# okgarces/deep-successor-features-for-transfer

Hardware: AMD Instinct MI355X
Metric: env steps/sec (whole node), Reacher 8-task SF-DQN at 1/2/4/8 MI355X (higher is better)
Workload: dtype fp32; 1 GPU; reacher17-all-T8-B32 (Reacher-shape |s|=17 |a|=7 d=8, psi MLP 256x2, all heads updated per env step: main_sfdqn_torch.py path); heads_per_gpu=8, heads_total=8, global_batch=32, replay=host, parallelism=single

## Files before the change

deep-successor-features-for-transfer_amd/csrc/sfx.hip:

```cpp
#include <hip/hip_ext.h>
#include <hip/hip_runtime.h>
#include <dlfcn.h>
#include <rccl/rccl.h>

#include <cmath>
#include <cstdio>
#include <cstdlib>
#include <cstring>
#include <algorithm>
#include <atomic>
#include <chrono>
#include <deque>
#include <map>
#include <random>
#include <string>
#include <functional>
#include <tuple>
#include <utility>
#include <vector>

#include "sfx_kernels.h"
#include "sfx_gpiw.h"
#include "sfx_tsf.h"
#include "sfx_phi.h"
// ... 38 lines not shown
      all = all && f != nullptr;
    };
    sym(a.GetUniqueId, "ncclGetUniqueId");
    sym(a.CommInitRank, "ncclCommInitRank");
    sym(a.AllReduce, "ncclAllReduce");
    sym(a.CommDestroy, "ncclCommDestroy");
    sym(a.CommAbort, "ncclCommAbort");
    sym(a.CommGetAsyncError, "ncclCommGetAsyncError");
    sym(a.CommSplit, "ncclCommSplit");
    sym(a.CommCount, "ncclCommCount");
    sym(a.CommUserRank, "ncclCommUserRank");
    sym(a.GetErrorString, "ncclGetErrorString");
    a.ok = all;
    if (!all) a.why = "RCCL lacks a needed entry point";
    return a;
  }();
  return api;
}

#define SFX_FAIL(code, msg) \
  do {                      \
    g_err = (msg);          \
    return (code);          \
  } while (0)

#define HIPCHK(x)                                                     \
  do {                                                                \
    hipError_t e_ = (x);                                              \
    if (e_ != hipSuccess) {                                           \
      g_err = std::string(#x) + ": " + hipGetErrorString(e_);         \
      return SFX_E_HIP;                                               \
    }                                                                 \
  } while (0)

#define LAUNCHCHK()                                                   \
  do {                                                                \
    hipError_t e_ = hipGetLastError();                                \
    if (e_ != hipSuccess) {                                           \
      g_err = std::string("kernel launch: ") + hipGetErrorString(e_); \
      return SFX_E_HIP;                                               \
    }                                                                 \
  } while (0)

#define RC(x)            \
  do {                   \
    int rc_ = (x);       \
    if (rc_) return rc_; \
  } while (0)

namespace {

inline int align4(int x) { return (x + 3) & ~3; }
inline int align8(int x) { return (x + 7) & ~7; }
inline int cdiv(int a, int b) { return (a + b - 1) / b; }

struct GraphKey {
  int op, a0, a1, a2, a3, a4, a5, a6;
  unsigned long long mask;
  const void* p[12];
  bool operator<(const GraphKey& o) const { return std::memcmp(this, &o, sizeof(GraphKey)) < 0; }
};

struct StepOut {
  int64_t sel[2];
  int flag;
  unsigned done;
  int posted;
  int pad_;
};

}

struct sfx_handle {
  int T = 0, n_s = 0, H = 0, nh = 0, A = 0, d = 0, O = 0, NL = 0, Mmax = 0, device = 0;
  int P = 0, Ptorch = 0, dpad = 0, actSize = 0;
  std::vector<LayerGeo> L;
  std::vector<int> actOff;
  hipStream_t stream = nullptr;
  hipStream_t cap = nullptr;
  bool use_graphs = true;
  int fwd_tpw = FWD_TPW;
  SelScratch* selk = nullptr;
  int ncu = 256;
  AdamHP hp_psi{1e-3, 0.0, 0.9, 0.999, 1e-8};
  AdamHP hp_w{1e-3, 0.0, 0.9, 0.999, 1e-8};
  int target_update_ev = 1000;
  std::vector<int> since_target, host_step;
  unsigned long long mask = 0;
  std::map<GraphKey, hipGraphExec_t> graphs;
  std::map<GraphKey, bool> graph_posts;
  std::map<GraphKey, int> keys_seen;
  long long graph_eager = 0;
  Geo G{};
  bool prof = false;
  struct ProfRec {
    int kind;
    double bytes;
    hipEvent_t a, b;
  };
  std::vector<ProfRec> prof_recs;
  std::vector<hipEvent_t> prof_pool;
  bool lazy_finish = false;
  struct Pending {
    bool active = false, update = false, sel = false;
    int B = 0, use_gpi = 1, task = 0, sel_use_gpi = 1;
    const float *S = nullptr, *S1 = nullptr, *phi = nullptr, *gamma = nullptr, *s_next = nullptr;
    const int64_t* a = nullptr;
    float* losses = nullptr;
    bool pre = false;
    const float* ax = nullptr;
    int aM = 0;
    bool posted = false;
    float* q_out = nullptr;
    int64_t* task_out = nullptr;
    const unsigned long long* out_ind = nullptr;
  } pend;
  long long steps_spec = 0, steps_fallback = 0, policies_rerun = 0, rounds_total = 0;
  long long graph_captures = 0, graph_launches = 0;
  int force_rerun_from = -1;
  int spec_rounds = 2;
  bool spec_rounds_auto = true;
  int Tg = 0, off = 0;
  struct sfx_tsf_state* tsf = nullptr;
  struct sfx_phi_state* phi = nullptr;
  int comm_rank = 0, comm_world = 0;
  ncclComm_t comm = nullptr;
  bool comm_owned = false;
  ncclComm_t comm_rounds = nullptr;
  bool rounds_comm = false;
  bool comm_dead = false;
  std::string comm_err;
  long long* dstall = nullptr;
  bool comm_force = false;
  int (*host_ar)(void*, int32_t*, int) = nullptr;
  void* host_ar_ctx = nullptr;
  int32_t* host_ar_buf = nullptr;
  size_t host_ar_cap = 0;
  int *xb[2] = {nullptr, nullptr}, *xge = nullptr;
  int *tsx = nullptr, *tsz = nullptr;
  int *qh = nullptr, *qhs = nullptr;
  bool shard_qa = true;
  Pending spend;

  float *online = nullptr, *target = nullptr, *am = nullptr, *av = nullptr;
  float *w = nullptr, *wm = nullptr, *wv = nullptr;
  int* step = nullptr;
  int* dcancel = nullptr;
  AdamC* adamc = nullptr;
  float *act = nullptr, *dz = nullptr, *rowloss = nullptr;
  int64_t* spec_next = nullptr;
  int* skip = nullptr;
  unsigned long long* skipc = nullptr;
  bool skip_rounds = true;
  bool bwd_merge = true;
  int tdg_rows = 0;
  StepOut* dout = nullptr;
  HostResult* pub_res = nullptr;
  const long long* pub_dctr = nullptr;
  bool pub_folded = false;
  bool fold_publish = true;
  bool bf16 = false;
  __bf16* on16 = nullptr;
  __bf16* tg16 = nullptr;
  int dxs_max = 1, dx_ntile = 1;
  float* dxpart = nullptr;
  unsigned* dxctr = nullptr;
// ... 172 lines not shown
    F.K = L.K;
    F.act = L.actOut;
    F.wOff = L.wOff;
    F.bOff = L.bOff;
    F.xOff = l == 0 || l0 ? -1 : h->actOff[l - 1];
    F.yOff = h->actOff[l];
    F.w0Off = h->L[0].wOff;
    F.b0Off = h->L[0].bOff;
    F.K0 = h->L[0].K;
    F.y0Off = h->actOff[0];
    const bool first = l == ex.l0 || l0;
    F.lms_head = first ? ex.lms_head : -1;
    F.lms_phi = ex.lms_phi;
    F.lms_r = ex.lms_r;
    F.lms_r_ind = first ? ex.lms_r_ind : nullptr;
    F.lms_alpha = ex.lms_alpha;
    F.flag = first ? ex.flag : nullptr;
    F.flag_value = ex.flag_value;
    const bool qa = ex.qa_role >= 0 && l == h->NL - 1;
    const bool aligned = l > 0 || ((uintptr_t)xa % 16 == 0 && (uintptr_t)xb % 16 == 0);
    bool own = false;
    if (F.xcd)
      for (const FwdGroup& g : groups) own = own || (g.m > 0 && g.m != M);
    F.ntN = cdiv(L.N, 16);
    long tiles32 = 0;
    for (const FwdGroup& g : groups) tiles32 += (long)F.ntN * cdiv(own && g.m > 0 ? g.m : M, 32) * g.n;
    F.tail = !l0 && !qa && (L.K % 32) == 0 && aligned && own && tiles32 > h->ncu ? 1 : 0;
    F.ntM = fwd_row_tiles(M, F.tail);
    F.tpw = 1;
    long tiles = (long)F.ntN * F.ntM * ninst;
    F.rowsplit = 0;
    if (own) {
      int* mt[4] = {&F.mt0, &F.mt1, &F.mt2, &F.mt3};
      int gi = 0;
      F.ntMs = 0;
      tiles = 0;
      for (const FwdGroup& g : groups) {
        *mt[gi++] = fwd_row_tiles(g.m > 0 ? g.m : M, F.tail);
        F.ntMs += *mt[gi - 1];
        tiles += (long)F.ntN * *mt[gi - 1] * g.n;
      }
      F.rowsplit = 1;
    }
    if (qa) {
      F.qa_role = ex.qa_role;
      F.qa_Tg = h->Tg;
      F.qa_off = h->off;
      F.qa_M = ex.qa_M;
      F.qa_all = ex.qa_all;
      F.qa_ge = ex.qa_ge;
      F.qa_lt = ex.qa_lt;
      F.qa_sel = ex.qa_sel;
      F.qa_row = ex.qa_row;
      F.qa_task = ex.qa_task;
      F.qa_use_gpi = ex.qa_use_gpi;
      F.qh = ex.qh;
      F.qhs = ex.qhs;
    }
    if (!qa && h->fwd_tpw > 1 && F.ntN > 1 && 2 * tiles >= 3L * h->ncu && (tiles <= 4L * h->ncu || F.rowsplit) &&
        (l0 || ((L.K % 32) == 0 && aligned)))
      F.tpw = h->fwd_tpw;
    const int ntNb = cdiv(F.ntN, F.tpw);
    const dim3 grid = F.xcd ? dim3(8 * cdiv(h->T, 8) * ntNb * (F.rowsplit ? F.ntMs : F.ntM * F.ngroups))
                            : dim3(ntNb, ninst, F.ntM);
    double by = 0.0;
    for (const FwdGroup& g : groups) {
      const double m = g.m > 0 ? g.m : M;
      by += 4.0 * g.n * ((double)L.N * L.K + L.N + m * L.K + m * L.N);
      if (l0) by += 4.0 * g.n * ((double)h->L[0].N * h->L[0].K + h->L[0].N + m * h->L[0].K);
    }
    const bool tp2 = F.tpw > 1;
    const bool gemv = !l0 && !qa && M <= GEMV_M && L.N >= GEMV_N && L.K % 16 == 0 &&
                      (l > 0 || ((uintptr_t)xa % 16 == 0 && (uintptr_t)xb % 16 == 0));
    if (gemv) {
      launch(h, K_FWD, by, k_fwd_gemv, dim3(cdiv(L.N, 64), ninst), dim3(256), h->G, F);
    } else if (l0) {
      if (!(ex.ride_l0 && !F.xcd && ex.ride_l0(F, grid, by)))
        launch(h, K_FWD, by,
               tp2 ? (h->bf16 ? k_fwd<true, true, true, 2> : k_fwd<true, true, false, 2>)
                   : (h->bf16 ? k_fwd<true, true, true> : k_fwd<true, true>),
               grid, dim3(64 * FWD_WAVES), h->G, F);
    } else {
      const bool vec = (L.K % 32) == 0 && aligned;
      launch(h, K_FWD, by,
             !vec ? k_fwd<false, false>
                  : tp2 ? (h->bf16 ? k_fwd<true, false, true, 2> : k_fwd<true, false, false, 2>)
                        : (h->bf16 ? k_fwd<true, false, true> : k_fwd<true, false>),
             grid, dim3(64 * FWD_WAVES), h->G, F);
    }
  }
  LAUNCHCHK();
  return SFX_OK;
}

bool wide_gpi(const sfx_handle* h) {
  return (long)h->T * h->A > 256 && h->d % 4 == 0 && h->d <= 16 && h->A <= WAMAX;
}

#define SFX_WIDE(K) (h->d == 4 ? K<1> : h->d == 8 ? K<2> : h->d == 12 ? K<3> : K<4>)

int run_tdg(sfx_handle* h, int pol0, int npol, int guess, int M, int use_gpi, const int64_t* a, const float* phi,
            const float* gamma, int64_t* next, int next_stride, int* flag = nullptr, const int* xmax = nullptr,
            int poloff = 0, const float* dz_scale = nullptr, const int64_t* prev = nullptr, bool skip = false) {
  const double nt = use_gpi ? h->T : 1;
  const double by = 4.0 * npol * M * (nt * h->O + 2.0 * h->O + 2.0 * h->d + 4);
  if (use_gpi && !xmax && !dz_scale && wide_gpi(h)) {
    TdgwArgs W{};
    W.M = M;
    W.pol0 = pol0;
    W.npol = npol;
    W.guess = guess;
    W.next_stride = next_stride;
    W.flag_value = h->T;
    W.a = a;
    W.phi = phi;
    W.gamma = gamma;
    W.next = next;
    W.flag = flag;
    W.prev = skip ? prev : nullptr;
    W.skip = skip ? h->skip : nullptr;
    W.skipc = skip ? h->skipc : nullptr;
    launch(h, K_TDG, by, SFX_WIDE(k_tdgw), dim3(M, cdiv(npol, WPC)), dim3(256), h->G, W);
    LAUNCHCHK();
    return SFX_OK;
  }
  TdgArgs A{};
  A.dz_scale = dz_scale;
  A.xmax = xmax;
  A.poloff = poloff;
  A.M = M;
  A.use_gpi = use_gpi;
  A.pol0 = pol0;
  A.npol = npol;
  A.guess = guess;
  A.flag = flag;
  A.flag_value = h->T;
  A.next_stride = next_stride;
  A.a = a;
  A.phi = phi;
  A.gamma = gamma;
  A.next = next;
  A.prev = skip ? prev : nullptr;
  A.skip = skip ? h->skip : nullptr;
  A.skipc = skip ? h->skipc : nullptr;
  launch(h, K_TDG, by, k_tdg, dim3(M, npol), dim3(256), h->G, A);
  LAUNCHCHK();
  return SFX_OK;
}

struct TdgSpec {
  int use_gpi = 1, guess = R_S1, next_stride = 0;
  const int64_t* a = nullptr;
  const float* gamma = nullptr;
  int64_t* next = nullptr;
  int* flag = nullptr;
  const int* xmax = nullptr;
  int poloff = 0;
  const int* xi_src = nullptr;
  int* xi_dst = nullptr;
  int xi_copy = 0, xi_n = 0;
  const int64_t* prev = nullptr;
  bool skip = false;
  const float* dz_scale = nullptr;
};

int tdg_variant(const sfx_handle* h) {
  if ((h->d & 3) != 0 || h->O > TDG_ROWS_O || h->A > 128) return 0;
  const long ta = (long)h->T * h->A;
// ... 688 lines not shown
                          float* phi_copy, const int64_t* idx, const float* gam, int B, float* S, float* PHI, float* S1,
                          int64_t* A, float* G, int n_s, int d) {
  if (!rs || !rphi || !rs1 || !ra || j < 0 || !s || !phi || !s1 || !a || !idx || (!rg && !gam) || B < 1 || !S ||
      !PHI || !S1 || !A || !G || n_s < 1 || d < 1)
    SFX_FAIL(SFX_E_ARG, "sfx_replay_put_gather: bad arguments");
  const PutGather P{rs, rphi, rs1, ra, rg, j, s, phi, s1, a, s1_copy, phi_copy, idx, gam, S, PHI, S1, G, A, B, n_s, d};
  hipLaunchKernelGGL(k_replay_put_gather, dim3(B + 1), dim3(64), 0, (hipStream_t)stream, P);
  LAUNCHCHK();
  return SFX_OK;
}
const char* sfx_last_error(void) { return g_err.c_str(); }

int sfx_check_failures(long long* count, long long* first_host, int reset) {
  if (!count) SFX_FAIL(SFX_E_ARG, "null argument");
#ifdef SFX_CHECK
  unsigned n = 0;
  HIPCHK(hipDeviceSynchronize());
  HIPCHK(hipMemcpyFromSymbol(&n, HIP_SYMBOL(sfx::g_chk_n), sizeof(n)));
  if (first_host) HIPCHK(hipMemcpyFromSymbol(first_host, HIP_SYMBOL(sfx::g_chk_rec), sizeof(long long) * 32));
  if (reset) {
    const unsigned z = 0;
    HIPCHK(hipMemcpyToSymbol(HIP_SYMBOL(sfx::g_chk_n), &z, sizeof(z)));
  }
  *count = n;
#else
  (void)first_host;
  (void)reset;
  *count = -1;
#endif
  return SFX_OK;
}

#ifdef SFX_PROBE
int sfx_probe_dump(void* out_host, int max_recs) {
  unsigned n = 0;
  if (hipDeviceSynchronize() != hipSuccess) return -1;
  if (hipMemcpyFromSymbol(&n, HIP_SYMBOL(sfx::g_probe_n), sizeof(n)) != hipSuccess) return -1;
  if (n > sfx::PROBE_N) n = sfx::PROBE_N;
  if ((int)n > max_recs) n = (unsigned)max_recs;
  if (n && hipMemcpyFromSymbol(out_host, HIP_SYMBOL(sfx::g_probe), n * sizeof(sfx::ProbeRec)) != hipSuccess) return -1;
  const unsigned z = 0;
  if (hipMemcpyToSymbol(HIP_SYMBOL(sfx::g_probe_n), &z, sizeof(z)) != hipSuccess) return -1;
  return (int)n;
}
#endif

int sfx_create(sfx_t* out, int T, int n_s, int H, int n_hidden, const int* acts, int A, int d, int max_batch,
               int device, void* stream) {
  if (!out) SFX_FAIL(SFX_E_ARG, "out is null");
  *out = nullptr;
  if (T < 1 || T > 64 || n_s < 1 || H < 1 || n_hidden < 0 || n_hidden + 2 > NLMAX || A < 1 || d < 1 ||
      max_batch < 1)
    SFX_FAIL(SFX_E_ARG, "bad geometry (1 <= T <= 64 heads per handle)");
  if (d > DMAX || max_batch + 1 > MMAX || A > AMAX || (long)T * A > QMAX || (long)A * d > OMAX)
    SFX_FAIL(SFX_E_ARG, "geometry exceeds kernel limits (d<=256, batch<1024, A<=256, T*A<=8192, A*d<=4096)");
  for (int i = 0; i < n_hidden; ++i)
    if (!acts || acts[i] < ACT_NONE || acts[i] > ACT_TANH) SFX_FAIL(SFX_E_ARG, "bad activation code");
  HIPCHK(hipSetDevice(device));
  sfx_handle* h = new sfx_handle();
  h->T = T;
  h->n_s = n_s;
  h->H = H;
  h->nh = n_hidden;
  h->A = A;
  h->d = d;
  h->O = A * d;
  h->NL = n_hidden + 2;
  h->Mmax = max_batch;
  h->device = device;
  h->stream = (hipStream_t)stream;
  h->dpad = align4(d);
  const char* eg = std::getenv("SFX_GRAPHS");
  h->use_graphs = !(eg && eg[0] == '0');
  const char* efp = std::getenv("SFX_FOLD_PUBLISH");
  h->fold_publish = !(efp && efp[0] == '0');
  {
    int dev = 0, ncu = 0;
    if (hipGetDevice(&dev) == hipSuccess &&
        hipDeviceGetAttribute(&ncu, hipDeviceAttributeMultiprocessorCount, dev) == hipSuccess && ncu > 0)
      h->ncu = ncu;
  }
  const char* etp = std::getenv("SFX_FWD_TPW");
  h->fwd_tpw = etp && etp[0] == '1' ? 1 : FWD_TPW;
  const char* eqa = std::getenv("SFX_SHARD_QA");
  h->shard_qa = !(eqa && eqa[0] == '0');
  const char* esk = std::getenv("SFX_SKIP");
  h->skip_rounds = !(esk && esk[0] == '0');
  const char* ebm = std::getenv("SFX_BWD_MERGE");
  h->bwd_merge = !(ebm && ebm[0] == '0');
  const char* etr = std::getenv("SFX_TDG_ROWS");
  const int tr = etr ? std::atoi(etr) : 0;
  h->tdg_rows = tr == 16 || tr == 32 ? tr : 0;
  int off = 0, ptorch = 0;
  for (int l = 0; l < h->NL; ++l) {
    LayerGeo Lr{};
    if (l == 0) {
      Lr.N = H; Lr.K = n_s; Lr.actOut = ACT_NONE;
    } else if (l == h->NL - 1) {
      Lr.N = h->O; Lr.K = H; Lr.actOut = ACT_NONE;
    } else {
      Lr.N = H; Lr.K = H; Lr.actOut = acts[l - 1];
    }
    Lr.actIn = l > 0 ? h->L[l - 1].actOut : ACT_NONE;
    Lr.wOff = align8(off);
    off = Lr.wOff + Lr.N * Lr.K;
    Lr.bOff = align4(off);
    off = Lr.bOff + Lr.N;
    ptorch += Lr.N * Lr.K + Lr.N;
    h->L.push_back(Lr);
  }
  h->P = (off + 63) & ~63;
  h->Ptorch = ptorch;
  int aoff = 0;
  for (int l = 0; l < h->NL; ++l) {
    h->actOff.push_back(aoff);
    aoff += align4((max_batch + 1) * h->L[l].N);
  }
  h->actSize = (aoff + 63) & ~63;
  h->Tg = T;
  h->spec_rounds = auto_spec_rounds(T);
  h->since_target.assign(T, 0);
  h->host_step.assign(T, 0);

  const size_t headBytes = sizeof(float) * (size_t)T * h->P;
  const size_t wBytes = sizeof(float) * (size_t)T * h->dpad;
  int rc = SFX_OK;
  auto alloc = [&](void** p, size_t bytes) {
    if (rc != SFX_OK) return;
    if (hipMalloc(p, bytes) != hipSuccess || hipMemset(*p, 0, bytes) != hipSuccess) {
      g_err = "hipMalloc failed";
      rc = SFX_E_HIP;
    }
  };
  alloc((void**)&h->online, 2 * headBytes);
  alloc((void**)&h->target, headBytes);
  alloc((void**)&h->am, 2 * headBytes);
  alloc((void**)&h->av, 2 * headBytes);
  alloc((void**)&h->w, wBytes);
  alloc((void**)&h->wm, wBytes);
  alloc((void**)&h->wv, wBytes);
  alloc((void**)&h->step, sizeof(int) * T);
  alloc((void**)&h->dcancel, 64);
  alloc((void**)&h->adamc, sizeof(AdamC) * T);
  {
    int nmax = 0, kmax = 0;
    for (const LayerGeo& L : h->L) {
      nmax = std::max(nmax, L.N);
      kmax = std::max(kmax, L.K);
    }
    h->dxs_max = std::max(1, cdiv(nmax, DX_SPLIT_N));
    h->dx_ntile = cdiv(max_batch, 32) * cdiv(kmax, 16);
    if (h->dxs_max > 1) {
      alloc((void**)&h->dxpart, sizeof(float) * 512 * (size_t)T * h->dx_ntile * h->dxs_max);
      alloc((void**)&h->dxctr, sizeof(unsigned) * (size_t)T * h->dx_ntile);
    }
  }
  alloc((void**)&h->act, sizeof(float) * (size_t)NROLE * T * h->actSize);
  alloc((void**)&h->dz, sizeof(float) * (size_t)T * h->actSize);
  alloc((void**)&h->rowloss, sizeof(float) * (size_t)T * MMAX);
  alloc((void**)&h->spec_next, sizeof(int64_t) * 2 * (size_t)T * MMAX);
  alloc((void**)&h->skip, sizeof(int) * 2 * (size_t)T);
  alloc((void**)&h->skipc, 64);
  alloc((void**)&h->dout, sizeof(StepOut));
  alloc((void**)&h->selk, sizeof(SelScratch));
  if (rc == SFX_OK &&
      hipHostMalloc((void**)&h->hout, sizeof(StepOut), hipHostMallocCoherent | hipHostMallocMapped) != hipSuccess) {
// ... 640 lines not shown
```

deep-successor-features-for-transfer_amd/csrc/sfx_kernels.h:

```cpp
#pragma once
#include <hip/hip_runtime.h>
#include <stdint.h>

#include <type_traits>

namespace sfx {

typedef float floatx4 __attribute__((ext_vector_type(4)));

constexpr int NLMAX = 8;
constexpr int MT = 32;
constexpr int QMAX = 8192;
constexpr int OMAX = 4096;
constexpr int AMAX = 256;
constexpr int DMAX = 256;
constexpr int MMAX = 1024;
constexpr int KFUSE = 64;
constexpr int GEMV_N = 512;
constexpr int GEMV_M = 4;
constexpr int DX_SPLIT_N = 256;
constexpr int VFUSE = 4096;
constexpr int TQF = 4096;

enum { ACT_NONE = 0, ACT_RELU = 1, ACT_TANH = 2 };
// ... 312 lines not shown
    for (int k = 0; k < d; ++k) q = __builtin_fmaf(p[k], w[k], q);
    const int v = sortable(q);
    SFX_CHK(i < Tg && m0 + bl < F.qa_M && head < G.T, i, m0 + bl, head);
    const size_t o = ((size_t)i * F.qa_M + m0 + bl) * Aa + a;
    if (all) atomicMax(F.qa_all + o, v);
    if (ge) atomicMax(F.qa_ge + o, v);
    if (lt) atomicMax(F.qa_lt + o, v);
    if (F.qh) F.qh[(((size_t)head * Tg + i) * F.qa_M + m0 + bl) * Aa + a] = v;
  }
  const int rl = F.qa_row - m0;
  if ((F.qa_sel || F.qhs) && rl >= 0 && rl < 32 && (F.qa_use_gpi || tg == F.qa_task))
    for (int al = tid; al < na; al += nt) {
      const int a = a0 + al;
      if (a >= Aa) continue;
      const float* p = sT + rl * 16 + al * d;
      const float* w = sw + F.qa_task * d;
      float q = 0.f;
      for (int k = 0; k < d; ++k) q = __builtin_fmaf(p[k], w[k], q);
      const int v = sortable(q);
      if (F.qa_sel) F.qa_sel[(size_t)tg * Aa + a] = v;
      if (F.qhs) F.qhs[(size_t)head * Aa + a] = v;
    }
}

__device__ void q_replay(const Geo& G, const FwdArgs& F, int head, int tN, int tM) {
  const int d = G.d, Aa = G.A, Tg = F.qa_Tg, tid = threadIdx.x, nt = blockDim.x;
  const int n0 = tN * 16, m0 = tM * 32, na = 16 / d, a0 = n0 / d, tg = F.qa_off + head;
  const int mrows = F.qa_M - m0 < 32 ? F.qa_M - m0 : 32;
  const int per_i = (mrows > 0 ? mrows : 0) * na;
  for (int it = tid; it < Tg * per_i; it += nt) {
    const int i = it / per_i, rem = it - i * per_i, bl = rem / na, al = rem - bl * na, a = a0 + al;
    if (a >= Aa || !F.qa_lt || tg >= i) continue;
    const int v = F.qh[(((size_t)head * Tg + i) * F.qa_M + m0 + bl) * Aa + a];
    atomicMax(F.qa_lt + ((size_t)i * F.qa_M + m0 + bl) * Aa + a, v);
  }
  const int rl = F.qa_row - m0;
  if (F.qa_sel && rl >= 0 && rl < 32 && (F.qa_use_gpi || tg == F.qa_task))
    for (int al = tid; al < na; al += nt) {
      const int a = a0 + al;
      if (a < Aa) F.qa_sel[(size_t)tg * Aa + a] = F.qhs[(size_t)head * Aa + a];
    }
}

__device__ void lms_apply(float* w, const float* phi, const float* r, float alpha, int d, int cx) {
  __shared__ float s_p[DMAX];
  __shared__ float s_e;
  const int tid = threadIdx.x;
  const float wk = tid < d ? w[tid] : 0.f, pk = tid < d ? phi[tid] : 0.f;
  if (tid < d) s_p[tid] = __fmul_rn(pk, wk);
  __syncthreads();
  if (tid == 0) {
    float rf = 0.f;
    for (int k = 0; k < d; ++k) rf = __fadd_rn(rf, s_p[k]);
    s_e = __fmul_rn(alpha, __fsub_rn(r[0], rf));
  }
  __syncthreads();
  if (tid < d && !cx) w[tid] = __fadd_rn(wk, __fmul_rn(s_e, pk));
}

__device__ void lms_block(const Geo& G, const FwdArgs& F) {
  const float* r = F.lms_r_ind ? reinterpret_cast<const float*>(F.lms_r_ind[0]) : F.lms_r;
  lms_apply(G.w + (long long)F.lms_head * G.dpad, F.lms_phi, r, F.lms_alpha, G.d, step_cancelled(G.cancel));
}

constexpr int L0_KMAX = 64, L0_NMAX = 256;

__device__ __forceinline__ FwdGroup fwd_group(const FwdArgs& F, int& y) {
  int gs = 0;
  if (F.ngroups > 1 && y >= F.g0.n) { y -= F.g0.n; gs = 1; }
  if (F.ngroups > 2 && gs == 1 && y >= F.g1.n) { y -= F.g1.n; gs = 2; }
  if (F.ngroups > 3 && gs == 2 && y >= F.g2.n) { y -= F.g2.n; gs = 3; }
  auto pick = [gs](int a, int b, int c, int d) { return gs == 0 ? a : gs == 1 ? b : gs == 2 ? c : d; };
  FwdGroup g;
  g.role = pick(F.g0.role, F.g1.role, F.g2.role, F.g3.role);
  g.which = pick(F.g0.which, F.g1.which, F.g2.which, F.g3.which);
  g.xsel = pick(F.g0.xsel, F.g1.xsel, F.g2.xsel, F.g3.xsel);
  g.head0 = pick(F.g0.head0, F.g1.head0, F.g2.head0, F.g3.head0);
  g.n = pick(F.g0.n, F.g1.n, F.g2.n, F.g3.n);
  g.m = pick(F.g0.m, F.g1.m, F.g2.m, F.g3.m);
  g.noskip = pick(F.g0.noskip, F.g1.noskip, F.g2.noskip, F.g3.noskip);
  return g;
}

constexpr int FWD_TPW = 2;
constexpr int FWD_WAVES = 8;

__host__ __device__ __forceinline__ int fwd_row_tiles(int m, int tail) {
  return tail && m > 32 ? (m + 15) >> 5 : (m + 31) >> 5;
}

template <bool VEC, bool L0, bool BF = false, int TP = 1>
__device__ __forceinline__ void fwd_tile(const Geo& G, const FwdArgs& F, int y, int tN, int tM, float* sT = nullptr) {
  constexpr int TPW = TP;
  static_assert(TP == 1 || VEC, "several tiles per workgroup: vector tiles only");
  const int ntile = TP == 1 ? 1 : (F.ntN - tN < F.tpw ? F.ntN - tN : F.tpw);
  static_assert(!BF || VEC, "bf16 operands: vector tiles only");
  constexpr int KW = 256 / FWD_WAVES;
  constexpr int KL = KW / 4;
  const FwdGroup grp = fwd_group(F, y);
  const int head = grp.head0 + y;
  const int M = grp.m > 0 ? grp.m : F.M, N = F.N, K = F.K;
  if (tM >= fwd_row_tiles(M, F.tail)) return;
  const float* P = grp.which == P_TARGET ? G.target + (long long)head * G.P
                                         : G.online + G.slot_off(rslot(F.mask, head) ^ (grp.which == P_NEW), head);
  const float* X = F.xOff < 0 ? (grp.xsel == 1 ? F.xa : grp.xsel == 2 ? F.xb : F.xc) : G.actp(grp.role, head, F.xOff);
  float* Y = G.actp(grp.role, head, F.yOff);
  const int m0 = tM * 32;
  const int wave = threadIdx.x >> 6, lane = threadIdx.x & 63, r = lane & 15, g = lane >> 4;
  const int ma = m0 + r, mb = m0 + 16 + r, mc = m0 + 32 + r;
  const bool oka = ma < M, okb = mb < M;
  constexpr bool EXT = VEC && !L0;
  const bool ext = EXT && F.tail && M - m0 > 32;
  const bool okc = ext && mc < M;
  const float* Pw = P + F.wOff;
  const __bf16* Pw16 = nullptr;
  if constexpr (BF)
    Pw16 = (grp.which == P_TARGET ? G.tg16 + (long long)head * G.P
                                  : G.on16 + G.slot_off(rslot(F.mask, head) ^ (grp.which == P_NEW), head)) +
           F.wOff;
  const int Lx = threadIdx.x & 63;
  float biasv[TPW];
#pragma unroll
  for (int j = 0; j < TPW; ++j) {
    const int col = (tN + j) * 16 + (Lx & 15);
    biasv[j] = (j < ntile && threadIdx.x < (ext ? 192 : 128) && col < N) ? *(P + F.bOff + col) : 0.f;
  }
  constexpr int AS = L0 ? L0_NMAX + 4 : 4;
  __shared__ __align__(16) float sA[L0 ? 32 * AS : 4];
  float4 wpre[TPW][VEC && L0 && !BF ? KL / 4 : 1];
  bf16x8 wpre16[TPW][BF && L0 ? KL / 8 : 1];
  if constexpr (VEC && L0 && !BF) {
    const int kb0 = wave * KW + g * KL;
#pragma unroll
    for (int j = 0; j < TPW; ++j) {
      const int nj = (tN + j) * 16 + r;
      const bool ok = j < ntile && nj < N && kb0 < K;
#pragma unroll
      for (int q = 0; q < KL / 4; ++q)
        wpre[j][q] = ok ? ld4(Pw + (size_t)nj * K + kb0 + 4 * q) : make_float4(0.f, 0.f, 0.f, 0.f);
    }
  }
  if constexpr (BF && L0) {
    const int kb0 = wave * KW + g * KL;
#pragma unroll
    for (int j = 0; j < TPW; ++j) {
      const int nj = (tN + j) * 16 + r;
      const bool ok = j < ntile && nj < N && kb0 < K;
#pragma unroll
      for (int q = 0; q < KL / 8; ++q) wpre16[j][q] = ok ? ld_bf16x8(Pw16 + (size_t)nj * K + kb0 + 8 * q) : bf16x8{};
    }
  }
  if constexpr (L0) {
    __shared__ float sX[32 * L0_KMAX];
    const int K0 = F.K0;
    const float* W0 = P + F.w0Off;
    const float* b0 = P + F.b0Off;
    float* Y0 = G.actp(grp.role, head, F.y0Off);
    constexpr int KS = L0_KMAX / 4;
    float wA[KS], wB[KS], bA, bB;
    auto load_w0 = [&](int cb) {
      const int nA = cb + r, nB = cb + 16 + r;
#pragma unroll
      for (int q = 0; q < KS; ++q) {
        const int kk = 4 * q + g;
        const bool okk = kk < K0;
        wA[q] = okk && nA < K ? W0[(size_t)nA * K0 + kk] : 0.f;
        wB[q] = okk && nB < K ? W0[(size_t)nB * K0 + kk] : 0.f;
      }
      bA = nA < K ? b0[nA] : 0.f;
      bB = nB < K ? b0[nB] : 0.f;
    };
    int cb = wave * 32;
    load_w0(cb);
    for (int j = threadIdx.x; j < 32 * K0; j += 64 * FWD_WAVES) {
      const int rr = j / fdiv(K0), kk = j - rr * K0;
      sX[j] = m0 + rr < M ? X[(size_t)(m0 + rr) * K0 + kk] : 0.f;
    }
    __syncthreads();
    PROBE_AT(3);
    for (; cb < K; cb += 32 * FWD_WAVES) {
      floatx4 c00 = {0.f, 0.f, 0.f, 0.f}, c01 = c00, c10 = c00, c11 = c00;
#pragma unroll
      for (int q = 0; q < KS; ++q) {
        if (4 * q < K0) {
          const int kk = 4 * q + g;
          const bool okk = kk < K0;
          const float x0 = okk ? sX[r * K0 + kk] : 0.f, x1 = okk ? sX[(16 + r) * K0 + kk] : 0.f;
          c00 = mfma4(x0, wA[q], c00);
          c01 = mfma4(x0, wB[q], c01);
          c10 = mfma4(x1, wA[q], c10);
          c11 = mfma4(x1, wB[q], c11);
        }
      }
      auto put = [&](const floatx4& c, int q) {
        const int cc = cb + (q & 1) * 16 + r;
        if (cc < K) {
          const float bb = (q & 1) ? bB : bA;
#pragma unroll
          for (int i = 0; i < 4; ++i) {
            const int rr = (q >> 1) * 16 + g * 4 + i;
            const float v = __fadd_rn(c[i], bb);
            sA[rr * AS + cc] = v;
            if (tN == 0 && m0 + rr < M) {
              G.chk_act(F.y0Off, (long long)(m0 + rr) * K + cc);
              Y0[(size_t)(m0 + rr) * K + cc] = v;
            }
          }
        }
      };
      put(c00, 0);
      put(c01, 1);
      put(c10, 2);
      put(c11, 3);
      if (cb + 32 * FWD_WAVES < K) load_w0(cb + 32 * FWD_WAVES);
    }
    __syncthreads();
    PROBE_AT(4);
  }
  const float* xra = L0 ? sA + r * AS : X + (size_t)ma * K;
  const float* xrb = L0 ? sA + (16 + r) * AS : X + (size_t)mb * K;
  const float* xrc = X + (size_t)(okc ? mc : 0) * K;
  __shared__ floatx4 red[FWD_WAVES][EXT ? 3 : 2][64];
  floatx4 acc0[TPW], acc1[TPW], acc2[EXT ? TPW : 1];
#pragma unroll
  for (int j = 0; j < TPW; ++j) acc0[j] = acc1[j] = floatx4{0.f, 0.f, 0.f, 0.f};
#pragma unroll
  for (int j = 0; j < (EXT ? TPW : 1); ++j) acc2[j] = floatx4{0.f, 0.f, 0.f, 0.f};
  const float* wrj[TPW];
  const __bf16* wr16j[TPW];
  bool oknj[TPW];
#pragma unroll
  for (int j = 0; j < TPW; ++j) {
    const int n = (tN + j) * 16 + r;
    oknj[j] = j < ntile && n < N;
    wrj[j] = Pw + (size_t)(oknj[j] ? n : 0) * K;
    wr16j[j] = BF ? Pw16 + (size_t)(oknj[j] ? n : 0) * K : nullptr;
  }
  for (int kc = wave * KW; kc < K && BF; kc += 256) {
    const int kb = kc + g * KL;
    float a0[KL], a1[KL], a2[EXT ? KL : 1];
#pragma unroll
    for (int q = 0; q < KL / 4; ++q) {
      float4 ta, tb;
      if constexpr (L0) {
        ta = reinterpret_cast<const float4*>(xra + kb)[q];
        tb = reinterpret_cast<const float4*>(xrb + kb)[q];
      } else {
        ta = oka ? *reinterpret_cast<const float4*>(xra + kb + 4 * q) : make_float4(0.f, 0.f, 0.f, 0.f);
        tb = okb ? *reinterpret_cast<const float4*>(xrb + kb + 4 * q) : make_float4(0.f, 0.f, 0.f, 0.f);
      }
      a0[4 * q] = ta.x; a0[4 * q + 1] = ta.y; a0[4 * q + 2] = ta.z; a0[4 * q + 3] = ta.w;
      a1[4 * q] = tb.x; a1[4 * q + 1] = tb.y; a1[4 * q + 2] = tb.z; a1[4 * q + 3] = tb.w;
      if constexpr (EXT) {
        const float4 tc = okc ? *reinterpret_cast<const float4*>(xrc + kb + 4 * q) : make_float4(0.f, 0.f, 0.f, 0.f);
        a2[4 * q] = tc.x; a2[4 * q + 1] = tc.y; a2[4 * q + 2] = tc.z; a2[4 * q + 3] = tc.w;
      }
    }
    bf16x8 w16[TPW][KL / 8];
#pragma unroll
    for (int j = 0; j < TPW; ++j)
#pragma unroll
      for (int q = 0; q < KL / 8; ++q) {
        if constexpr (L0)
          w16[j][q] = kc == wave * KW ? wpre16[j][q] : (oknj[j] ? ld_bf16x8(wr16j[j] + kb + 8 * q) : bf16x8{});
        else
          w16[j][q] = oknj[j] ? ld_bf16x8(wr16j[j] + kb + 8 * q) : bf16x8{};
      }
#pragma unroll
    for (int q = 0; q < KL / 8; ++q) {
      const bf16x8 x0 = to_bf16x8(a0 + 8 * q), x1 = to_bf16x8(a1 + 8 * q);
#pragma unroll
      for (int j = 0; j < TPW; ++j) {
        acc0[j] = mfma_bf16(x0, w16[j][q], acc0[j]);
        acc1[j] = mfma_bf16(x1, w16[j][q], acc1[j]);
      }
    }
    if constexpr (EXT)
      if (ext)
#pragma unroll
        for (int q = 0; q < KL / 8; ++q) {
          const bf16x8 x2 = to_bf16x8(a2 + 8 * q);
#pragma unroll
          for (int j = 0; j < TPW; ++j) acc2[j] = mfma_bf16(x2, w16[j][q], acc2[j]);
        }
  }
  for (int kc = wave * KW; kc < K && !BF; kc += 256) {
    const int kb = kc + g * KL;
    float a0[KL], a1[KL], bw[TPW][KL], a2[EXT ? KL : 1];
    if constexpr (VEC) {
#pragma unroll
      for (int q = 0; q < KL / 4; ++q) {
        float4 ta, tb;
        if constexpr (L0) {
          ta = reinterpret_cast<const float4*>(xra + kb)[q];
          tb = reinterpret_cast<const float4*>(xrb + kb)[q];
        } else {
          ta = oka ? ld4(xra + kb + 4 * q) : make_float4(0.f, 0.f, 0.f, 0.f);
          tb = okb ? ld4(xrb + kb + 4 * q) : make_float4(0.f, 0.f, 0.f, 0.f);
        }
#pragma unroll
        for (int j = 0; j < TPW; ++j) {
          float4 tw;
          if constexpr (L0 && !BF) {
            tw = kc == wave * KW ? wpre[j][q]
                                 : (oknj[j] ? ld4(wrj[j] + kb + 4 * q) : make_float4(0.f, 0.f, 0.f, 0.f));
          } else {
            tw = oknj[j] ? ld4(wrj[j] + kb + 4 * q) : make_float4(0.f, 0.f, 0.f, 0.f);
          }
          bw[j][4 * q] = tw.x; bw[j][4 * q + 1] = tw.y; bw[j][4 * q + 2] = tw.z; bw[j][4 * q + 3] = tw.w;
        }
        a0[4 * q] = ta.x; a0[4 * q + 1] = ta.y; a0[4 * q + 2] = ta.z; a0[4 * q + 3] = ta.w;
        a1[4 * q] = tb.x; a1[4 * q + 1] = tb.y; a1[4 * q + 2] = tb.z; a1[4 * q + 3] = tb.w;
        if constexpr (EXT) {
          const float4 tc = okc ? ld4(xrc + kb + 4 * q) : make_float4(0.f, 0.f, 0.f, 0.f);
          a2[4 * q] = tc.x; a2[4 * q + 1] = tc.y; a2[4 * q + 2] = tc.z; a2[4 * q + 3] = tc.w;
        }
      }
    } else {
#pragma unroll
      for (int i = 0; i < KL; ++i) {
        const bool kin = kb + i < K;
        if constexpr (L0) {
          a0[i] = (oka && kin) ? xra[kb + i] : 0.f;
          a1[i] = (okb && kin) ? xrb[kb + i] : 0.f;
        } else {
          a0[i] = (oka && kin) ? *(xra + kb + i) : 0.f;
          a1[i] = (okb && kin) ? *(xrb + kb + i) : 0.f;
        }
#pragma unroll
        for (int j = 0; j < TPW; ++j) bw[j][i] = (oknj[j] && kin) ? *(wrj[j] + kb + i) : 0.f;
      }
    }
#pragma unroll
    for (int i = 0; i < KL; ++i)
#pragma unroll
      for (int j = 0; j < TPW; ++j) {
        acc0[j] = mfma4(a0[i], bw[j][i], acc0[j]);
        acc1[j] = mfma4(a1[i], bw[j][i], acc1[j]);
      }
    if constexpr (EXT)
      if (ext)
#pragma unroll
        for (int i = 0; i < KL; ++i)
#pragma unroll
          for (int j = 0; j < TPW; ++j) acc2[j] = mfma4(a2[i], bw[j][i], acc2[j]);
  }
#pragma unroll
  for (int j = 0; j < TPW; ++j) {
  if (j >= ntile) continue;
  const int n0 = (tN + j) * 16, col = n0 + (Lx & 15);
  const float bias = biasv[j];
  PROBE_MARK();
  if (j > 0) __syncthreads();
  red[wave][0][lane] = acc0[j];
  red[wave][1][lane] = acc1[j];
  if constexpr (EXT)
    if (ext) red[wave][EXT ? 2 : 1][lane] = acc2[EXT ? j : 0];
  __syncthreads();
  if (threadIdx.x < (ext ? 192 : 128)) {
    const int s = threadIdx.x >> 6;
    floatx4 v = red[0][s][Lx];
#pragma unroll
    for (int w2 = 1; w2 < FWD_WAVES; ++w2) v += red[w2][s][Lx];
    if (col < N) {
#pragma unroll
      for (int i = 0; i < 4; ++i) {
        const int row = m0 + 16 * s + (Lx >> 4) * 4 + i;
        const float o = act_fwd(__fadd_rn(v[i], bias), F.act);
        if (row < M) {
          G.chk_act(F.yOff, (long long)row * N + col);
          Y[(size_t)row * N + col] = o;
        }
        if (sT) sT[(row - m0) * 16 + (col - n0)] = row < M ? o : 0.f;
      }
    }
  }
  }
}

constexpr int qa_tile_floats(bool L0) { return L0 ? 1 : 32 * 16; }

template <bool VEC, bool L0, bool BF, int TP>
__device__ __forceinline__ void fwd_body(const Geo& G, const FwdArgs& F, int bx, int by, int bz) {
  PROBE_T(pt0);
  int y = by, tN = bx, tM = bz;
  const int ntNb = TP > 1 ? (F.ntN + F.tpw - 1) / F.tpw : F.ntN;
  if (F.xcd) {
    const int b = bx, hp = (F.nh + 7) >> 3, k = b >> 3;
    const int r = hp == 1 ? k : k / fdiv(hp), hd = (b & 7) + 8 * (k - r * hp);
    const int rN = r / fdiv(ntNb);
    int gi;
    tN = r - rN * ntNb;
    if (F.rowsplit) {
      tM = rN;
      gi = 0;
      if (tM >= F.mt0) {
        tM -= F.mt0;
        gi = 1;
        if (tM >= F.mt1) {
          tM -= F.mt1;
          gi = 2;
          if (tM >= F.mt2) {
            tM -= F.mt2;
            gi = 3;
          }
        }
      }
    } else {
      gi = rN / fdiv(F.ntM);
      tM = rN - gi * F.ntM;
    }
    if (hd >= F.nh || gi >= F.ngroups) return;
    y = gi * F.nh + hd;
  }
  if constexpr (TP > 1) tN *= F.tpw;
  bool qa = false;
  int head = 0;
  if (F.qa_role >= 0) {
    int yy = y;
    const FwdGroup grp = fwd_group(F, yy);
    qa = grp.role == F.qa_role;
    head = grp.head0 + yy;
  }
  if (F.skip) {
    int yy = y;
    const FwdGroup grp = fwd_group(F, yy);
    if (!grp.noskip && __builtin_nontemporal_load(F.skip + grp.head0 + yy)) {
      if (qa && F.qh) q_replay(G, F, head, tN, tM);
      return;
    }
  }
  __shared__ float sT[qa_tile_floats(L0)];
  fwd_tile<VEC, L0, BF, TP>(G, F, y, tN, tM, qa ? sT : nullptr);
  if (qa) q_accumulate(G, F, head, tN, tM, sT);
  if (tN == 0 && tM == 0 && by == 0 && (F.xcd ? bx == 0 : true)) {
    if (F.flag && threadIdx.x == 0) *F.flag = F.flag_value;
    if (F.lms_head >= 0) lms_block(G, F);
  }
  PROBE_REC(L0 ? 2 : 1, pt0);
}

template <bool VEC, bool L0, bool BF = false, int TP = 1>
__global__ __launch_bounds__(64 * FWD_WAVES) void k_fwd(Geo G, FwdArgs F) {
  fwd_body<VEC, L0, BF, TP>(G, F, blockIdx.x, blockIdx.y, blockIdx.z);
}

__global__ __launch_bounds__(256) void k_fwd_gemv(Geo G, FwdArgs F) {
  PROBE_T(pt0);
  int y = blockIdx.y;
  const FwdGroup grp = fwd_group(F, y);
  const int head = grp.head0 + y;
  if (F.skip && __builtin_nontemporal_load(F.skip + head)) return;
  const int M = F.M, N = F.N, K = F.K;
  const float* P = grp.which == P_TARGET ? G.target + (long long)head * G.P
                                         : G.online + G.slot_off(rslot(F.mask, head) ^ (grp.which == P_NEW), head);
  const float* X = F.xOff < 0 ? (grp.xsel == 1 ? F.xa : grp.xsel == 2 ? F.xb : F.xc) : G.actp(grp.role, head, F.xOff);
  float* Y = G.actp(grp.role, head, F.yOff);
  const int wave = threadIdx.x >> 6, lane = threadIdx.x & 63, q = lane & 3;
  const int n = blockIdx.x * 64 + wave * 16 + (lane >> 2);
  const bool okn = n < N;
  const float* wr = P + F.wOff + (size_t)(okn ? n : 0) * K;
  float acc[GEMV_M];
#pragma unroll
  for (int m = 0; m < GEMV_M; ++m) acc[m] = 0.f;
  for (int kc = 0; kc < K; kc += 256) {
    float4 wv[16];
#pragma unroll
    for (int i = 0; i < 16; ++i) {
      const int k = kc + 16 * i + 4 * q;
      wv[i] = k < K ? *reinterpret_cast<const float4*>(wr + k) : make_float4(0.f, 0.f, 0.f, 0.f);
    }
#pragma unroll
    for (int m = 0; m < GEMV_M; ++m) {
      if (m < M) {
        const float* xr = X + (size_t)m * K;
#pragma unroll
        for (int i = 0; i < 16; ++i) {
          const int k = kc + 16 * i + 4 * q;
          const float4 xv = k < K ? *reinterpret_cast<const float4*>(xr + k) : make_float4(0.f, 0.f, 0.f, 0.f);
          acc[m] = __builtin_fmaf(xv.x, wv[i].x, acc[m]);
          acc[m] = __builtin_fmaf(xv.y, wv[i].y, acc[m]);
          acc[m] = __builtin_fmaf(xv.z, wv[i].z, acc[m]);
          acc[m] = __builtin_fmaf(xv.w, wv[i].w, acc[m]);
        }
      }
    }
  }
  const float bias = okn ? P[F.bOff + n] : 0.f;
#pragma unroll
  for (int m = 0; m < GEMV_M; ++m) {
    float v = acc[m];
    v = __fadd_rn(v, __int_as_float(__builtin_amdgcn_update_dpp(0, __float_as_int(v), 0xB1, 0xF, 0xF, false)));
    v = __fadd_rn(v, __int_as_float(__builtin_amdgcn_update_dpp(0, __float_as_int(v), 0x4E, 0xF, 0xF, false)));
    if (m < M && okn && q == 0) Y[(size_t)m * N + n] = act_fwd(__fadd_rn(v, bias), F.act);
  }
  PROBE_REC(19, pt0);
}

__device__ __forceinline__ float td_norm(const Geo& G, int M, int O, const float* dz_scale) {
  const float n = (float)((G.huber > 0.f ? 1.0 : 2.0) / ((double)M * (double)O));
  return dz_scale ? __fmul_rn(n, *dz_scale) : n;
}
__device__ __forceinline__ float td_grad(float huber, float norm, float x) {
  if (huber > 0.f) {
    const float nd = __fmul_rn(norm, huber);
    return x < -huber ? -nd : (x > huber ? nd : __fmul_rn(norm, x));
  }
  return __fmul_rn(norm, x);
}
__device__ __forceinline__ float td_loss(float huber, float x) {
  if (huber > 0.f) {
    const float z = fabsf(x);
    return z < huber ? __fmul_rn(__fmul_rn(0.5f, z), z) : __fmul_rn(huber, __fsub_rn(z, __fmul_rn(0.5f, huber)));
  }
  return __fmul_rn(x, x);
}

__device__ __forceinline__ void tdg_skip_report(int* skip, unsigned long long* skipc, int pol, int T, bool differs,
                                                bool have_prev, int nrep) {
  int* word = skip + T + pol;
  const int old = __hip_atomic_fetch_add(word, differs ? 0x10001 : 1, __ATOMIC_RELAXED, __HIP_MEMORY_SCOPE_AGENT);
  if ((old & 0xFFFF) == nrep - 1) {
    const bool any = (old >> 16) != 0 || differs;
    skip[pol] = any ? 0 : 1;
    if (skipc && have_prev) {
      atomicAdd(skipc, 1ull);
      if (!any) atomicAdd(skipc + 1, 1ull);
// ... 500 lines not shown
    return;
  }
  if (threadIdx.x < NRED) {
    const floatx4 v = dx_red_sum(red, s, Lx);
    if (col < K) {
#pragma unroll
      for (int i = 0; i < 4; ++i) {
        const int row = m0 + 16 * s + (Lx >> 4) * 4 + i;
        if (row < M) {
          G.chk_act(L.dzIn, (long long)row * K + col);
          out[(size_t)row * K + col] = act_bwd(v[i], xin[i], L.actIn);
        }
      }
    }
  }
}

__device__ __forceinline__ int v0_aoff(const BwdArgs& A, int K) { return (A.vM * K + 3) & ~3; }
constexpr int V0S = KFUSE + 4;

__device__ __forceinline__ void v0_tile(const float* x, int K, int m0, int rows, const float* w, float bb, int act,
                                        float* Y, int N, int n, long long lim) {
  constexpr int KS = 8;
  const int lane = threadIdx.x & 63, r = lane & 15, g = lane >> 4, ma = m0 + r;
  floatx4 c = {0.f, 0.f, 0.f, 0.f};
  for (int k0 = 0; k0 < K; k0 += 4 * KS) {
    float a[KS], b[KS];
#pragma unroll
    for (int q = 0; q < KS; ++q) {
      const int k = k0 + 4 * q + g;
      a[q] = (k < K && ma < rows) ? x[ma * K + k] : 0.f;
      b[q] = k < K ? w[k] : 0.f;
    }
#pragma unroll
    for (int q = 0; q < KS; ++q)
      if (k0 + 4 * q < K) c = mfma4(a[q], b[q], c);
  }
  if (n < N) {
#pragma unroll
    for (int i = 0; i < 4; ++i) {
      const int m = m0 + g * 4 + i;
      if (m < rows) {
        SFX_CHK((long long)m * N + n < lim, m, n, lim);
        Y[(size_t)m * N + n] = act_fwd(__fadd_rn(c[i], bb), act);
      }
    }
  }
}

template <int NW = 32>
__device__ __forceinline__ void fused_v0(const Geo& G, const BwdArgs& A, const RoleGeo& L, int head, int nbase, const float* sW,
                         const float* sB, const float* sX, const float* sWt = nullptr, const float* sBt = nullptr,
                         bool vrows = true, bool landed = false) {
  if (A.aM > 0 && !landed) asm volatile("s_waitcnt vmcnt(0)" ::: "memory");
  __syncthreads();
  PROBE_AT(3);
  const int K = L.K, N = L.N, VM = A.vM;
  static_assert(NW == 16 || NW == 32, "layer-0 tile width");
  constexpr int WS = NW == 32 ? 2 : 4;
  const int wave = threadIdx.x >> 6, lane = threadIdx.x & 63, r = lane & 15;
  const int wt = NW == 32 ? wave >> 1 : wave;
  const int nl = (NW == 32 ? (wave & 1) * 16 : 0) + r, n = nbase + nl;
  const float bias = sB[nl];
  if (vrows) {
    float* Y = G.actp(A.vRole, head, A.vOff);
    for (int mt = wt; mt * 16 < VM; mt += WS)
      v0_tile(sX, K, mt * 16, VM, sW + nl * V0S, bias, A.act0, Y, N, n, G.actSize - A.vOff);
  }
  PROBE_AT(4);
  if (A.aM > 0) {
    const int aM = A.aM, nt = (aM + 15) >> 4;
    const float* xa = sX + v0_aoff(A, K);
    const float bt = sBt[nl];
    for (int it = wt; it < 3 * nt; it += WS) {
      const int which = it / nt, mt = it - which * nt;
      v0_tile(xa + (which ? aM * K : 0), K, mt * 16, aM, which == 2 ? sWt + nl * K : sW + nl * V0S,
              which == 2 ? bt : bias, A.act0, G.actp(which == 0 ? R_NS : which == 1 ? R_NS1 : R_NS1T, head, A.vOff),
              N, n, G.actSize - A.vOff);
    }
  }
  PROBE_AT(5);
}

typedef __attribute__((address_space(3))) void* tsf_lds_t;

template <class F>
__device__ __forceinline__ void glds(float* dst, int n, F src, int w0 = 0, int nw = 4) {
  const int lane = threadIdx.x & 63, wv = (threadIdx.x >> 6) - w0;
  if (wv < 0 || wv >= nw) return;
  for (int c = wv; c * 64 < n; c += nw) {
    const int j = c * 64 + lane;
    const float* p = j < n ? src(j) : nullptr;
    if (p)
      __builtin_amdgcn_global_load_lds((const void*)p, (tsf_lds_t)(dst + c * 64), 4, 0, 0);
    else if (j < n)
      dst[j] = 0.f;
  }
}

template <int NW = 32>
struct V0Smem {
  float sW[NW * V0S];
  float sB[NW];
  float sWt[NW * KFUSE];
  float sBt[NW];
  __align__(16) float sX[VFUSE];
};
template <int NW = 32>
__device__ __forceinline__ V0Smem<NW>& v0_smem() {
  __shared__ V0Smem<NW> sm;
  return sm;
}

template <int NW>
__device__ __forceinline__ void v0_stage_ahead(const Geo& G, const BwdArgs& A, const RoleGeo& L, int head, int nbase,
                                               V0Smem<NW>& sm) {
  const int K = L.K, ncol = L.N - nbase < NW ? L.N - nbase : NW;
  const float* ax = A.ax;
  glds(sm.sX + v0_aoff(A, K), 2 * A.aM * K, [&](int j) -> const float* { return ax + j; });
  const float* Pt = G.target + (long long)head * G.P;
  const float* tw = Pt + L.wOff + (size_t)nbase * K;
  glds(sm.sWt, NW * K, [&](int j) -> const float* { return j < ncol * K ? tw + j : nullptr; });
  const float* tb = Pt + L.bOff + nbase;
  glds(sm.sBt, NW, [&](int j) -> const float* { return j < ncol ? tb + j : nullptr; }, 0, 1);
}

template <int NW = 32>
__device__ __forceinline__ void role_v0_only(const Geo& G, const BwdArgs& A, int head, const RoleGeo& L, int tile, bool vrows) {
  const int N = L.N, K = L.K, M = A.M, tid = threadIdx.x, nbase = tile * NW;
  const float* Pw = G.online + G.slot_off(rslot(A.mask, head) ^ 1, head);
  V0Smem<NW>& sm = v0_smem<NW>();
  float* sW = sm.sW;
  float* sB = sm.sB;
  float* sX = sm.sX;
  if (A.aM > 0) v0_stage_ahead(G, A, L, head, nbase, sm);
  const FDiv fK = fdiv(K);
  for (int j = tid; j < NW * K; j += 256) {
    const int nl = j / fK, k = j - nl * K;
    sW[nl * V0S + k] = nbase + nl < N ? Pw[L.wOff + (size_t)(nbase + nl) * K + k] : 0.f;
  }
  if (tid < NW) sB[tid] = nbase + tid < N ? Pw[L.bOff + nbase + tid] : 0.f;
  if (vrows) {
    const int nxs = A.vM * K;
    for (int j = tid; j < nxs; j += 256) sX[j] = j < M * K ? A.v_x[j] : A.v_xn[j - M * K];
  }
  fused_v0<NW>(G, A, L, head, nbase, sW, sB, sX, sm.sWt, sm.sBt, vrows);
}

template <bool BF = false, bool MG = false>
__device__ __forceinline__ void role_dw(const Geo& G, const BwdArgs& A, int head, const RoleGeo& L, int tile, bool fuse,
                                        floatx4 (*red)[2][64] = nullptr) {
  constexpr int NW = MG ? 16 : 32;
  constexpr int NH = MG ? 1 : 2;
  const int N = L.N, K = L.K, M = A.M;
  const int ntk = (K + 63) >> 6;
  const int kt = tile % ntk, nt = tile / ntk;
  const int wave = threadIdx.x >> 6, lane = threadIdx.x & 63, r = lane & 15, g = lane >> 4;
  const int nbase = nt * NW, n0 = MG ? nbase : nbase + (wave & 1) * 16;
  const int k0 = kt * 64 + (MG ? wave * 16 : (wave >> 1) * 32);
  const float* dZ = G.dzp(head, L.dzOff);
  const float* X = layer_input(G, A, head, L.xOff);
  const int rs = rslot(A.mask, head);
  const long long ro = G.slot_off(rs, head), wo = G.slot_off(rs ^ 1, head);
  const float* Pr = G.online + ro;
  const float* Mr = G.am + ro;
  const float* Vr = G.av + ro;
  float* Pw = G.online + wo;
  float* Mw = G.am + wo;
// ... 1204 lines not shown
```

Before: 9271 env steps/s.

## Stage fp32 forward-tile operands into LDS via direct global-to-LDS loads

Adds an STG variant of the hidden-layer forward tile kernel. Each wave copies its activation rows and weight rows for a K-chunk into a swizzled per-wave LDS buffer using global_load_lds, then reads float4 fragments from LDS instead of issuing per-lane global vector loads. It is enabled by default for fp32 vector tiles when the grid has no more workgroups than CUs, and can be turned off with SFX_FWD_STAGE=0. The aim is more coalesced, wider memory transactions for small-batch launches, at the cost of a large per-block LDS allocation and a full waitcnt stall before compute.

```diff
diff --git a/deep-successor-features-for-transfer_amd/csrc/sfx.hip b/deep-successor-features-for-transfer_amd/csrc/sfx.hip
--- a/deep-successor-features-for-transfer_amd/csrc/sfx.hip
+++ b/deep-successor-features-for-transfer_amd/csrc/sfx.hip
@@ -144,6 +144,7 @@
   int fwd_tpw = FWD_TPW;
   SelScratch* selk = nullptr;
   int ncu = 256;
+  bool fwd_stage = true;
   AdamHP hp_psi{1e-3, 0.0, 0.9, 0.999, 1e-8};
   AdamHP hp_w{1e-3, 0.0, 0.9, 0.999, 1e-8};
   int target_update_ev = 1000;
@@ -482,8 +483,11 @@
                grid, dim3(64 * FWD_WAVES), h->G, F);
     } else {
       const bool vec = (L.K % 32) == 0 && aligned;
+      const long nwg = (long)grid.x * grid.y * grid.z;
+      const bool stg = vec && !h->bf16 && nwg <= h->ncu && h->fwd_stage;
       launch(h, K_FWD, by,
              !vec ? k_fwd<false, false>
+                  : stg ? (tp2 ? k_fwd<true, false, false, 2, true> : k_fwd<true, false, false, 1, true>)
                   : tp2 ? (h->bf16 ? k_fwd<true, false, true, 2> : k_fwd<true, false, false, 2>)
                         : (h->bf16 ? k_fwd<true, false, true> : k_fwd<true, false>),
              grid, dim3(64 * FWD_WAVES), h->G, F);
@@ -1338,6 +1342,8 @@
   }
   const char* etp = std::getenv("SFX_FWD_TPW");
   h->fwd_tpw = etp && etp[0] == '1' ? 1 : FWD_TPW;
+  const char* efs = std::getenv("SFX_FWD_STAGE");
+  h->fwd_stage = !(efs && efs[0] == '0');
   const char* eqa = std::getenv("SFX_SHARD_QA");
   h->shard_qa = !(eqa && eqa[0] == '0');
   const char* esk = std::getenv("SFX_SKIP");
diff --git a/deep-successor-features-for-transfer_amd/csrc/sfx_kernels.h b/deep-successor-features-for-transfer_amd/csrc/sfx_kernels.h
--- a/deep-successor-features-for-transfer_amd/csrc/sfx_kernels.h
+++ b/deep-successor-features-for-transfer_amd/csrc/sfx_kernels.h
@@ -418,6 +418,9 @@
   return g;
 }
 
+typedef __attribute__((address_space(3))) void* tsf_lds_t;
+__device__ __forceinline__ int stg_swz(int r) { return (r >> 1) ^ ((r >= 4 && r < 12) ? 2 : 0); }
+
 constexpr int FWD_TPW = 2;
 constexpr int FWD_WAVES = 8;
 
@@ -425,12 +428,13 @@
   return tail && m > 32 ? (m + 15) >> 5 : (m + 31) >> 5;
 }
 
-template <bool VEC, bool L0, bool BF = false, int TP = 1>
+template <bool VEC, bool L0, bool BF = false, int TP = 1, bool STG = false>
 __device__ __forceinline__ void fwd_tile(const Geo& G, const FwdArgs& F, int y, int tN, int tM, float* sT = nullptr) {
   constexpr int TPW = TP;
   static_assert(TP == 1 || VEC, "several tiles per workgroup: vector tiles only");
   const int ntile = TP == 1 ? 1 : (F.ntN - tN < F.tpw ? F.ntN - tN : F.tpw);
   static_assert(!BF || VEC, "bf16 operands: vector tiles only");
+  static_assert(!STG || (VEC && !L0 && !BF), "staged operands: plain fp32 vector tiles only");
   constexpr int KW = 256 / FWD_WAVES;
   constexpr int KL = KW / 4;
   const FwdGroup grp = fwd_group(F, y);
@@ -557,6 +561,8 @@
   const float* xrb = L0 ? sA + (16 + r) * AS : X + (size_t)mb * K;
   const float* xrc = X + (size_t)(okc ? mc : 0) * K;
   __shared__ floatx4 red[FWD_WAVES][EXT ? 3 : 2][64];
+  constexpr int SROWS = 16 * (3 + TP);
+  __shared__ __align__(16) float sStg[STG ? FWD_WAVES * SROWS * KW : 4];
   floatx4 acc0[TPW], acc1[TPW], acc2[EXT ? TPW : 1];
 #pragma unroll
   for (int j = 0; j < TPW; ++j) acc0[j] = acc1[j] = floatx4{0.f, 0.f, 0.f, 0.f};
@@ -623,7 +629,45 @@
   for (int kc = wave * KW; kc < K && !BF; kc += 256) {
     const int kb = kc + g * KL;
     float a0[KL], a1[KL], bw[TPW][KL], a2[EXT ? KL : 1];
-    if constexpr (VEC) {
+    if constexpr (STG) {
+      float* ws = sStg + wave * SROWS * KW;
+      const float4 z4 = make_float4(0.f, 0.f, 0.f, 0.f);
+      PROBE_AT(4);
+#pragma unroll
+      for (int i = 0; i < SROWS / 8; ++i) {
+        const int blk = i >> 1, rr = 8 * (i & 1) + (lane >> 3);
+        const float* src;
+        if (blk < 3) {
+          if (blk == 2 && !ext) continue;
+          const int m = m0 + 16 * blk + rr;
+          src = X + (size_t)(m < M ? m : 0) * K;
+        } else {
+          if (blk - 3 >= ntile) continue;
+          const int n = (tN + blk - 3) * 16 + rr;
+          src = Pw + (size_t)(n < N ? n : 0) * K;
+        }
+        __builtin_amdgcn_global_load_lds((const void*)(src + kc + 4 * ((lane & 7) ^ stg_swz(rr))), (tsf_lds_t)(ws + 256 * i),
+                                         16, 0, 0);
+      }
+      __builtin_amdgcn_s_waitcnt(0);
+      __builtin_amdgcn_fence(__ATOMIC_ACQUIRE, "wavefront");
+      PROBE_AT(3);
+      const float* wr = ws + r * KW;
+#pragma unroll
+      for (int q = 0; q < KL / 4; ++q) {
+        const int p4 = 4 * ((2 * g + q) ^ stg_swz(r));
+        const float4 ta = oka ? ld4(wr + p4) : z4, tb = okb ? ld4(wr + 16 * KW + p4) : z4;
+        const float4 tc = okc ? ld4(wr + 32 * KW + p4) : z4;
+#pragma unroll
+        for (int j = 0; j < TPW; ++j) {
+          const float4 tw = oknj[j] ? ld4(wr + (48 + 16 * j) * KW + p4) : z4;
+          bw[j][4 * q] = tw.x; bw[j][4 * q + 1] = tw.y; bw[j][4 * q + 2] = tw.z; bw[j][4 * q + 3] = tw.w;
+        }
+        a0[4 * q] = ta.x; a0[4 * q + 1] = ta.y; a0[4 * q + 2] = ta.z; a0[4 * q + 3] = ta.w;
+        a1[4 * q] = tb.x; a1[4 * q + 1] = tb.y; a1[4 * q + 2] = tb.z; a1[4 * q + 3] = tb.w;
+        a2[4 * q] = tc.x; a2[4 * q + 1] = tc.y; a2[4 * q + 2] = tc.z; a2[4 * q + 3] = tc.w;
+      }
+    } else if constexpr (VEC) {
 #pragma unroll
       for (int q = 0; q < KL / 4; ++q) {
         float4 ta, tb;
@@ -716,9 +760,10 @@
 
 constexpr int qa_tile_floats(bool L0) { return L0 ? 1 : 32 * 16; }
 
-template <bool VEC, bool L0, bool BF, int TP>
+template <bool VEC, bool L0, bool BF, int TP, bool STG = false>
 __device__ __forceinline__ void fwd_body(const Geo& G, const FwdArgs& F, int bx, int by, int bz) {
   PROBE_T(pt0);
+  PROBE_MARKA();
   int y = by, tN = bx, tM = bz;
   const int ntNb = TP > 1 ? (F.ntN + F.tpw - 1) / F.tpw : F.ntN;
   if (F.xcd) {
@@ -767,7 +812,7 @@
     }
   }
   __shared__ float sT[qa_tile_floats(L0)];
-  fwd_tile<VEC, L0, BF, TP>(G, F, y, tN, tM, qa ? sT : nullptr);
+  fwd_tile<VEC, L0, BF, TP, STG>(G, F, y, tN, tM, qa ? sT : nullptr);
   if (qa) q_accumulate(G, F, head, tN, tM, sT);
   if (tN == 0 && tM == 0 && by == 0 && (F.xcd ? bx == 0 : true)) {
     if (F.flag && threadIdx.x == 0) *F.flag = F.flag_value;
@@ -776,9 +821,9 @@
   PROBE_REC(L0 ? 2 : 1, pt0);
 }
 
-template <bool VEC, bool L0, bool BF = false, int TP = 1>
+template <bool VEC, bool L0, bool BF = false, int TP = 1, bool STG = false>
 __global__ __launch_bounds__(64 * FWD_WAVES) void k_fwd(Geo G, FwdArgs F) {
-  fwd_body<VEC, L0, BF, TP>(G, F, blockIdx.x, blockIdx.y, blockIdx.z);
+  fwd_body<VEC, L0, BF, TP, STG>(G, F, blockIdx.x, blockIdx.y, blockIdx.z);
 }
 
 __global__ __launch_bounds__(256) void k_fwd_gemv(Geo G, FwdArgs F) {
@@ -1445,8 +1490,6 @@
   PROBE_AT(5);
 }
 
-typedef __attribute__((address_space(3))) void* tsf_lds_t;
-
 template <class F>
 __device__ __forceinline__ void glds(float* dst, int n, F src, int w0 = 0, int nw = 4) {
   const int lane = threadIdx.x & 63, wv = (threadIdx.x >> 6) - w0;
```

Result: faster. 9365 env steps/s, median of 5 (+1.0%).
